# Rikorose/DeepFilterNet

Hardware: NVIDIA H100
Metric: 48kHz audio-sec/sec (batched enhance) (higher is better)
Workload: dtype f32 (bf16x3 tensor-core contractions, fp32 accumulate; DSP and gates IEEE fp32)

## Files before the change

### deepfilternet_b200/_lib.py

```python
from __future__ import annotations

import ctypes as C
import os
import subprocess

_HERE = os.path.dirname(os.path.abspath(__file__))
SO_PATH = os.path.join(_HERE, "libdfb200.so")

DFB_ERR_INVALID, DFB_ERR_CUDA, DFB_ERR_UNSUPPORTED, DFB_ERR_OOM = -1, -2, -3, -4


class DfbError(RuntimeError):
    def __init__(self, code: int, msg: str):
        super().__init__(msg)
        self.code = code


class ModelConfigC(C.Structure):
    _fields_ = [(n, C.c_int32) for n in (
        "model_kind", "nb_erb", "nb_df", "df_order", "df_lookahead", "conv_lookahead", "conv_ch",
        "conv_kt", "inp_kt", "emb_hidden", "df_hidden", "enc_gru_layers", "erb_gru_layers",
        "df_gru_layers", "df_pathway_kt", "enc_concat", "g_df_fc_emb", "g_enc_in", "g_enc_out",
        "g_erb_in", "g_erb_out", "g_df_in", "g_df_skip", "g_df_out")] + [
        ("lsnr_scale", C.c_float), ("lsnr_offset", C.c_float), ("norm_alpha", C.c_float)]


class TensorC(C.Structure):
    _fields_ = [("name", C.c_char_p), ("data", C.POINTER(C.c_float)), ("numel", C.c_int64)]


def build(force: bool = False) -> str:
    src_dir = os.path.join(_HERE, "csrc")
    if force and os.path.exists(SO_PATH):
        os.remove(SO_PATH)
    subprocess.check_call(["make", "-C", src_dir, "-j4"], stdout=subprocess.DEVNULL)
    return SO_PATH


_lib = None

_VP, _FP, _I64, _I, _F = C.c_void_p, C.POINTER(C.c_float), C.c_int64, C.c_int, C.c_float
_I64P = C.POINTER(C.c_int64)

SIGNATURES = {
    "dfb_last_error": (C.c_char_p, []),
    "dfb_version": (C.c_char_p, []),
    "dfb_kernel_launches": (_I64, []),
    "dfb_profile_enable": (_I, [_I, C.c_char_p]),
    "dfb_profile_report": (_I64, [C.c_char_p, _I64]),
    "dfb_state_create": (_I, [C.POINTER(_VP), _I, _I, _I, _I, _I, _I]),
    "dfb_state_free": (None, [_VP]),
    "dfb_state_erb_widths": (_I, [_VP, _I64P]),
    "dfb_state_fft_window": (_I, [_VP, _FP]),
    "dfb_state_params": (_I, [_VP, C.POINTER(_I), C.POINTER(_I), C.POINTER(_I), C.POINTER(_I)]),
    "dfb_erb_widths": (_I, [_I, _I, _I, _I, _I64P]),
    "dfb_analysis": (_I, [_VP, _VP, _I64, _I64, _VP, _VP]),
    "dfb_analysis_host": (_I, [_VP, _VP, _I64, _I64, _VP]),
    "dfb_analysis_host_ex": (_I, [_VP, _VP, _I64, _I64, _I, _VP]),
    "dfb_synthesis_host_ex": (_I, [_VP, _VP, _I64, _I64, _I, _VP]),
    "dfb_state_reset": (_I, [_VP]),
    "dfb_synthesis": (_I, [_VP, _VP, _I64, _I64, _VP, _VP]),
    "dfb_synthesis_host": (_I, [_VP, _VP, _I64, _I64, _VP]),
    "dfb_erb_host": (_I, [_I, _VP, _I64, _I64, _I64P, _I, _I, _VP]),
    "dfb_erb_inv_host": (_I, [_I, _VP, _I64, _I64P, _I, _VP]),
    "dfb_erb_norm_host": (_I, [_I, _VP, _I64, _I64, _I64, _F, _VP, _VP]),
    "dfb_unit_norm_host": (_I, [_I, _VP, _I64, _I64, _I64, _F, _VP, _VP]),
    "dfb_unit_norm_init": (_I, [_I64, _VP]),
    "dfb_features": (_I, [_VP, _VP, _I64, _I64, _I, _F, _VP, _VP, _VP, _VP]),
    "dfb_features_host": (_I, [_VP, _VP, _I64, _I64, _I, _F, _VP, _VP, _VP]),
    "dfb_resample_host": (_I, [_I, _VP, _I64, _I64, _VP, _I, _I, _I, _VP, _I64]),
    "dfb_model_create": (_I, [C.POINTER(_VP), _I, C.POINTER(ModelConfigC), C.POINTER(TensorC), _I, _I64P]),
    "dfb_model_free": (None, [_VP]),
    "dfb_model_forward": (_I, [_VP, _VP, _VP, _I64, _I64, _VP, _VP, _VP, _VP, _VP]),
    "dfb_apply": (_I, [_VP, _VP, _VP, _VP, _VP, _I64, _I64, _VP, _VP]),
    "dfb_model_forward_full": (_I, [_VP, _VP, _VP, _VP, _VP, _I64, _I64, _VP, _VP, _VP, _VP, _VP, _VP]),
    "dfb_enhance": (_I, [_VP, _VP, _VP, _I64, _I64, _I, _F, _VP, _VP]),
    "dfb_enhance_host": (_I, [_VP, _VP, _VP, _I64, _I64, _I, _F, _VP]),
    "dfb_enhance_out_len": (_I64, [_VP, _I64, _I]),
    "dfb_enhance_ragged": (_I, [_VP, _VP, _VP, _I64, _VP, _VP, _I64, _I, _F, _VP, _I64, _VP, _VP]),
    "dfb_enhance_ragged_host": (_I, [_VP, _VP, _VP, _I64, _VP, _VP, _I64, _I, _F, _VP, _I64, _VP]),
    "dfb_enhance_ragged_linked": (_I, [_VP, _VP, _VP, _I64, _VP, _VP, _I64, _I, _F, _VP, _I64, _VP, _VP, _I64, _I, _VP]),
    "dfb_enhance_ragged_linked_host": (_I, [_VP, _VP, _VP, _I64, _VP, _VP, _I64, _I, _F, _VP, _I64, _VP, _VP, _I64, _I]),
    "dfb_model_workspace_bytes": (_I64, [_VP]),
    "dfb_stream_create": (_I, [C.POINTER(_VP), _VP, _VP, _I64, _F]),
    "dfb_stream_free": (None, [_VP]),
    "dfb_stream_reset": (_I, [_VP]),
    "dfb_stream_frame_length": (_I64, [_VP]),
    "dfb_stream_latency_frames": (_I64, [_VP]),
    "dfb_stream_set_lsnr_thresholds": (_I, [_VP, _I, _F, _F, _F]),
    "dfb_stream_set_mask_reduce": (_I, [_VP, _I, _I]),
    "dfb_stream_process": (_I, [_VP, _VP, _I64, _VP, _VP]),
    "dfb_stream_flush": (_I, [_VP, _VP, _VP]),
    "dfb_stream_process_host": (_I, [_VP, _VP, _I64, _VP]),
    "dfb_stream_open_slots": (_I, [_VP, _I64P, _I64]),
    "dfb_stream_close_slots": (_I, [_VP, _I64P, _I64]),
    "dfb_stream_slot_states": (_I, [_VP, C.POINTER(C.c_int32)]),
    "dfb_stream_open_linked": (_I, [_VP, _I64P, _I64]),
    "dfb_stream_slot_groups": (_I, [_VP, _I64P]),
    "dfb_stream_set_atten_lim": (_I, [_VP, _I64P, _I64, _F]),
    "dfb_stream_set_post_filter_beta": (_I, [_VP, _I64P, _I64, _F]),
    "dfb_stream_process_lsnr": (_I, [_VP, _VP, _I64, _VP, _VP, _VP]),
    "dfb_stream_flush_lsnr": (_I, [_VP, _VP, _VP, _VP]),
    "dfb_stream_process_host_lsnr": (_I, [_VP, _VP, _I64, _VP, _VP]),
    "dfb_model_set_max_workspace": (_I, [_VP, _I64]),
    "dfb_model_set_options": (_I, [_VP, _I, _F, _I]),
    "dfb_model_set_chunking": (_I, [_VP, _I, _I, _I]),
    "dfb_debug_gru_timing": (_I, [_VP, _I, _VP]),
    "dfb_model_debug_fetch": (_I64, [_VP, C.c_char_p, _VP, _I64]),
}


def lib() -> C.CDLL:
    global _lib
    if _lib is None:
        if not os.path.exists(SO_PATH):
            raise ImportError(
                f"{SO_PATH} is missing: build it with `python -c 'import __graft_entry__ as g; g.build()'` "
                "(nvcc, sm_90a).  deepfilternet_b200 has no CPU fallback.")
        L = C.CDLL(SO_PATH)
        for name, (res, args) in SIGNATURES.items():
            fn = getattr(L, name)
            fn.restype = res
            fn.argtypes = args
        _lib = L
    return _lib


def check(rc: int) -> None:
    if rc != 0:
        msg = lib().dfb_last_error()
        raise DfbError(rc, (msg or b"unknown error").decode())
```

### deepfilternet_b200/csrc/dfb_gl.cu

```cuda
#include <cuda.h>
#include <cuda_bf16.h>

#include <map>
#include <mutex>
#include <tuple>

#include "dfb_common.cuh"
#include "dfb_dwpw.cuh"
#include "dfb_ptx.cuh"

namespace dfb {

constexpr int kGxThreads = 288, kGxMaxStages = 6, kGxBoxBytes = 128 * 128 ;
constexpr int kGxMaxChunks = 16;

struct GlBxParams {
    const unsigned short *w_img;
    const float *res; int64_t ldr;
    float *y; int64_t ldy;
    unsigned short *y_hi, *y_lo; int64_t ldp;
    int M, G, Ig, Hg, Hgp, gpc, act, stages;
    float oscale, ooffset;
};

__device__ __forceinline__ float gx_act(float x, int act) {
    if (act == 1) return fmaxf(x, 0.f);
    if (act == 2) return gt_tanh(x);
    return x;
}

__device__ __noinline__ void gl_store_chunk(const GlBxParams &p, int c, int g0, int cpg, int64_t mrow, int lane, float a00, float a01,
                                            float a02, float a03, float a10, float a11, float a12, float a13) {
    const float a[2][4] = {{a00, a01, a02, a03}, {a10, a11, a12, a13}};
    const int gl = c / cpg;
#pragma unroll
    for (int j = 0; j < 2; j++) {
        const int n = (c - gl * cpg) * 16 + j * 8 + 2 * (lane & 3);
        if (n >= p.Hg) continue;
        const int64_t col = (int64_t)(g0 + gl) * p.Hg + n;
        float2 rv[2];
#pragma unroll
        for (int h = 0; h < 2; h++) {
            const int64_t m = mrow + 8 * h;
            rv[h] = (p.res && m < p.M) ? *reinterpret_cast<const float2 *>(p.res + m * p.ldr + col) : make_float2(0.f, 0.f);
        }
#pragma unroll
        for (int h = 0; h < 2; h++) {
            const int64_t m = mrow + 8 * h;
            if (m >= p.M) continue;
            float2 x;
            x.x = gx_act(a[j][2 * h], p.act) * p.oscale + p.ooffset + rv[h].x;
            x.y = gx_act(a[j][2 * h + 1], p.act) * p.oscale + p.ooffset + rv[h].y;
            if (p.y) *reinterpret_cast<float2 *>(p.y + m * p.ldy + col) = x;
            if (p.y_hi) {
                uint32_t hv, lv;
                bf16x2_split(x.x, x.y, hv, lv);
                *reinterpret_cast<uint32_t *>(p.y_hi + m * p.ldp + col) = hv;
                *reinterpret_cast<uint32_t *>(p.y_lo + m * p.ldp + col) = lv;
            }
        }
    }
}

__global__ void __launch_bounds__(kGxThreads, 1)
k_gl_bx(const __grid_constant__ CUtensorMap tmXhi, const __grid_constant__ CUtensorMap tmXlo, const __grid_constant__ GlBxParams p) {
    extern __shared__ __align__(1024) unsigned char gx_smem_raw[];
    const uint32_t sb = (smem_u32(gx_smem_raw) + 1023u) & ~1023u;
    const int warp = threadIdx.x >> 5, lane = threadIdx.x & 31;
    const int slice = blockIdx.x, g0 = slice * p.gpc;
    const int nch = p.gpc * p.Hgp / 16;
    const int cpg = p.Hgp / 16;
    const int nboxes = p.gpc * p.Ig / 64;
    const int ntiles = (p.M + 127) / 128;
    const uint32_t gbytes = (uint32_t)p.Ig * p.Hgp * 2;
    const uint32_t wplane = gbytes * p.gpc;
    const uint32_t lbo = (uint32_t)(p.Hgp / 8) * 128u;
    const uint32_t s_x = sb;
    const uint32_t s_w = s_x + (uint32_t)p.stages * 2 * kGxBoxBytes;
    const uint32_t s_bar = (s_w + 2 * wplane + 127u) & ~127u;
    const uint32_t b_full = s_bar, b_empty = s_bar + 8 * kGxMaxStages, b_w = b_empty + 8 * kGxMaxStages;
    if (threadIdx.x == 0) {
        for (int s = 0; s < p.stages; s++) { mbar_init_a(b_full + 8 * s, 1); mbar_init_a(b_empty + 8 * s, 8); }
        mbar_init_a(b_w, 1);
        fence_barrier_init();
        mbar_expect_tx_a(b_w, 2 * wplane);
        const unsigned char *src = reinterpret_cast<const unsigned char *>(p.w_img);
        bulk_load(s_w, src + (size_t)g0 * gbytes, wplane, b_w);
        bulk_load(s_w + wplane, src + (size_t)p.G * gbytes + (size_t)g0 * gbytes, wplane, b_w);
    }
    __syncthreads();
    if (warp == 8) {
        if (lane == 0) {
            tma_prefetch_desc(&tmXhi); tma_prefetch_desc(&tmXlo);
            const int col0 = g0 * p.Ig;
            int it = 0;
            for (int tile = blockIdx.y; tile < ntiles; tile += gridDim.y)
                for (int b = 0; b < nboxes; b++, it++) {
                    const int s = it % p.stages, n = it / p.stages;
                    if (n > 0) mbar_wait_a(b_empty + 8 * s, (uint32_t)((n - 1) & 1));
                    mbar_expect_tx_a(b_full + 8 * s, 2 * kGxBoxBytes);
                    const uint32_t dst = s_x + (uint32_t)s * 2 * kGxBoxBytes;
                    asm volatile(
                        "cp.async.bulk.tensor.2d.shared::cluster.global.mbarrier::complete_tx::bytes [%0], [%1, {%2, %3}], [%4];"
                        ::"r"(dst), "l"((uint64_t)&tmXhi), "r"(col0 + b * 64), "r"(tile * 128), "r"(b_full + 8 * s) : "memory");
                    asm volatile(
                        "cp.async.bulk.tensor.2d.shared::cluster.global.mbarrier::complete_tx::bytes [%0], [%1, {%2, %3}], [%4];"
                        ::"r"(dst + kGxBoxBytes), "l"((uint64_t)&tmXlo), "r"(col0 + b * 64), "r"(tile * 128), "r"(b_full + 8 * s) : "memory");
                }
        }
        return;
    }
    const int mat = lane >> 3, rr = lane & 7;
    mbar_wait_a(b_w, 0);
    int it = 0;
    for (int tile = blockIdx.y; tile < ntiles; tile += gridDim.y) {
        float acc[kGxMaxChunks][2][4];
#pragma unroll
        for (int c = 0; c < kGxMaxChunks; c++)
#pragma unroll
            for (int e = 0; e < 8; e++) acc[c][e >> 2][e & 3] = 0.f;
        for (int b = 0; b < nboxes; b++, it++) {
            const int s = it % p.stages, n = it / p.stages;
            mbar_wait_a(b_full + 8 * s, (uint32_t)(n & 1));
            const uint32_t xs = s_x + (uint32_t)s * 2 * kGxBoxBytes;
#pragma unroll 1
            for (int k = 0; k < 4; k++) {
                const int col = b * 64 + k * 16;
                const int gl = col / p.Ig, kk = (col - gl * p.Ig) >> 4;
                uint32_t ah[4], al[4];
                const int r = warp * 16 + rr + ((mat & 1) << 3);
                ldsm_x4(xs + sw128_off(r, 2 * k + (mat >> 1)), ah);
                ldsm_x4(xs + kGxBoxBytes + sw128_off(r, 2 * k + (mat >> 1)), al);
                const uint32_t wa = s_w + (uint32_t)gl * gbytes + (uint32_t)(2 * kk + (mat & 1)) * lbo + (uint32_t)rr * 16u;
#pragma unroll
                for (int c = 0; c < kGxMaxChunks; c++) {
                    const int cg = c - gl * cpg;
                    if (c >= nch || cg < 0 || cg >= cpg) continue;
                    const uint32_t o = wa + (uint32_t)(2 * cg + (mat >> 1)) * 128u;
                    uint32_t bh[4], bl[4];
                    ldsm_x4(o, bh);
                    ldsm_x4(o + wplane, bl);
                    mma_bf16x3(acc[c][0], ah, al, bh[0], bh[1], bl[0], bl[1]);
                    mma_bf16x3(acc[c][1], ah, al, bh[2], bh[3], bl[2], bl[3]);
                }
            }
            __syncwarp();
            if (lane == 0) mbar_arrive_a(b_empty + 8 * s);
        }
        const int64_t mrow = (int64_t)tile * 128 + warp * 16 + (lane >> 2);
#pragma unroll
        for (int c = 0; c < kGxMaxChunks; c++)
            if (c < nch)
                gl_store_chunk(p, c, g0, cpg, mrow, lane, acc[c][0][0], acc[c][0][1], acc[c][0][2], acc[c][0][3], acc[c][1][0],
                               acc[c][1][1], acc[c][1][2], acc[c][1][3]);
    }
}

constexpr int kDeThreads = 288, kDeMaxStages = 6, kDeMaxChunks = 4;
constexpr uint32_t kDeBin = 32768;

struct DfEmbParams {
    const float *dw;
    const float *bias;
    const float *pw_sw;
    const unsigned short *w_img;
    const float *res; int64_t ldr;
    unsigned short *y_hi, *y_lo; int64_t ldp;
    int M, T, G, Ig, Hg, Hgp, S, stages;
    float oscale, ooffset;
    const int64_t *first;
    int64_t w0;
};

template <int KT>
__global__ void __launch_bounds__(kDeThreads, 1)
k_dwpw_gl(const __grid_constant__ CUtensorMap tmC0, const __grid_constant__ DfEmbParams p) {
    extern __shared__ __align__(1024) unsigned char de_smem_raw[];
    const uint32_t sb = (smem_u32(de_smem_raw) + 1023u) & ~1023u;
    const int warp = threadIdx.x >> 5, lane = threadIdx.x & 31;
    constexpr int RT = 128 - (KT - 1);
    const int ntiles = (p.M + RT - 1) / RT;
    const int j0 = blockIdx.x * p.S;
    const int f_lo = j0 > 0 ? 2 * j0 - 1 : 0, f_hi = 2 * (j0 + p.S);
    const int gps = p.S * kCh / p.Ig, cpg = p.Hgp / 16, nch = gps * cpg;
    const int g0 = j0 * kCh / p.Ig;
    const uint32_t gbytes = (uint32_t)p.Ig * p.Hgp * 2;
    const uint32_t wplane = gbytes * gps;
    const uint32_t lbo = (uint32_t)(p.Hgp / 8) * 128u;
    const uint32_t s_c0 = sb;
    const uint32_t s_pw = s_c0 + (uint32_t)p.stages * kDeBin;
    const uint32_t s_w = s_pw + 2u * kCh * 128u;
    const uint32_t s_bias = s_w + 2 * wplane;
    const uint32_t s_dw = s_bias + 256u;
    const uint32_t s_bar = (s_dw + KT * 3 * kCh * 4u + 127u) & ~127u;
    const uint32_t b_full = s_bar, b_empty = s_bar + 8 * kDeMaxStages, b_w = b_empty + 8 * kDeMaxStages;
    if (threadIdx.x == 0) {
        for (int s = 0; s < p.stages; s++) { mbar_init_a(b_full + 8 * s, 1); mbar_init_a(b_empty + 8 * s, 8); }
        mbar_init_a(b_w, 1);
        fence_barrier_init();
        mbar_expect_tx_a(b_w, 2u * kCh * 128u + 2 * wplane);
        bulk_load(s_pw, p.pw_sw, 2u * kCh * 128u, b_w);
        const unsigned char *src = reinterpret_cast<const unsigned char *>(p.w_img);
        bulk_load(s_w, src + (size_t)g0 * gbytes, wplane, b_w);
        bulk_load(s_w + wplane, src + (size_t)p.G * gbytes + (size_t)g0 * gbytes, wplane, b_w);
    }
    if (threadIdx.x < kCh / 4) sts128(s_bias + threadIdx.x * 16, __ldg(reinterpret_cast<const float4 *>(p.bias) + threadIdx.x));
    for (int i = threadIdx.x; i < KT * 3 * kCh / 4; i += kDeThreads) sts128(s_dw + i * 16, __ldg(reinterpret_cast<const float4 *>(p.dw) + i));
    __syncthreads();
    if (warp == 8) {
        if (lane == 0) {
            tma_prefetch_desc(&tmC0);
            int it = 0;
            for (int tile = blockIdx.y; tile < ntiles; tile += gridDim.y) {
                const int row0 = tile * RT - (KT - 1);
                for (int f = f_lo; f < f_hi; f++, it++) {
                    const int s = it % p.stages, n = it / p.stages;
                    if (n > 0) mbar_wait_a(b_empty + 8 * s, (uint32_t)((n - 1) & 1));
                    mbar_expect_tx_a(b_full + 8 * s, kDeBin);
                    const uint32_t dst = s_c0 + (uint32_t)s * kDeBin;
                    asm volatile(
                        "cp.async.bulk.tensor.2d.shared::cluster.global.mbarrier::complete_tx::bytes [%0], [%1, {%2, %3}], [%4];"
                        ::"r"(dst), "l"((uint64_t)&tmC0), "r"(f * kCh), "r"(row0), "r"(b_full + 8 * s) : "memory");
                    asm volatile(
                        "cp.async.bulk.tensor.2d.shared::cluster.global.mbarrier::complete_tx::bytes [%0], [%1, {%2, %3}], [%4];"
                        ::"r"(dst + kDeBin / 2), "l"((uint64_t)&tmC0), "r"(f * kCh + 32), "r"(row0), "r"(b_full + 8 * s) : "memory");
                }
            }
        }
        return;
    }
    const int g = lane >> 2, q = lane & 3, mat = lane >> 3, rr = lane & 7;
    mbar_wait_a(b_w, 0);
    int it = 0;
    for (int tile = blockIdx.y; tile < ntiles; tile += gridDim.y, it += f_hi - f_lo) {
        const int row0 = tile * RT - (KT - 1);
        bool tap_ok[2][KT];
#pragma unroll
        for (int rs = 0; rs < 2; rs++) {
            const int r = warp * 16 + g + 8 * rs, m = row0 + r;
#pragma unroll
            for (int dt = 0; dt < KT; dt++) tap_ok[rs][dt] = true;
            if (KT > 1) {
                const int b = m >= 0 && m < p.M ? m / p.T : 0, t = m - b * p.T;
                const int t_first = stream_first(p.first, b, p.w0);
#pragma unroll
                for (int dt = 0; dt < KT; dt++) tap_ok[rs][dt] = r - (KT - 1) + dt >= 0 && t - (KT - 1 - dt) >= t_first;
            }
        }
        float gacc[kDeMaxChunks][2][4];
#pragma unroll
        for (int c = 0; c < kDeMaxChunks; c++)
#pragma unroll
            for (int e = 0; e < 8; e++) gacc[c][e >> 2][e & 3] = 0.f;
        for (int jj = 0; jj < p.S; jj++) {
            const int j = j0 + jj;
            uint32_t slot[3];
#pragma unroll
            for (int df = 0; df < 3; df++) {
                const int f = 2 * j - 1 + df;
                const int i = it + (f < f_lo ? 0 : f - f_lo);
                slot[df] = s_c0 + (uint32_t)(i % p.stages) * kDeBin;
                if (f >= f_lo) mbar_wait_a(b_full + 8 * (i % p.stages), (uint32_t)((i / p.stages) & 1));
            }
            uint32_t ah[4][4], al[4][4];
#pragma unroll
            for (int ks = 0; ks < 4; ks++)
#pragma unroll
                for (int h = 0; h < 2; h++) {
                    const int ch = 16 * ks + 8 * h + 2 * q;
                    const uint32_t cbase = (uint32_t)(ch >> 5) * (kDeBin / 2) + (uint32_t)(ch & 3) * 4u;
                    const int chunk = (ch & 31) >> 2;
#pragma unroll
                    for (int rs = 0; rs < 2; rs++) {
                        const int r = warp * 16 + g + 8 * rs;
                        float2 acc = make_float2(0.f, 0.f);
#pragma unroll
                        for (int dt = 0; dt < KT; dt++) {
                            if (!tap_ok[rs][dt]) continue;
                            const int rb = r - (KT - 1) + dt;
                            const uint32_t o = cbase + (uint32_t)rb * 128u + (uint32_t)((chunk ^ (rb & 7)) << 4);
#pragma unroll
                            for (int df = 0; df < 3; df++) {
                                if (df == 0 && j == 0) continue;
                                float2 x;
                                asm volatile("ld.shared.v2.f32 {%0, %1}, [%2];" : "=f"(x.x), "=f"(x.y) : "r"(slot[df] + o));
                                float2 w;
                                asm volatile("ld.shared.v2.f32 {%0, %1}, [%2];" : "=f"(w.x), "=f"(w.y) : "r"(s_dw + 4u * ((dt * 3 + df) * kCh + ch)));
                                acc.x = fmaf(x.x, w.x, acc.x);
                                acc.y = fmaf(x.y, w.y, acc.y);
                            }
                        }
                        bf16x2_split(acc.x, acc.y, ah[ks][rs + 2 * h], al[ks][rs + 2 * h]);
                    }
                }
            __syncwarp();
            if (lane == 0) {
                for (int f = 2 * j - 1; f <= 2 * j + (jj + 1 == p.S ? 1 : 0); f++)
                    if (f >= f_lo) mbar_arrive_a(b_empty + 8 * ((it + f - f_lo) % p.stages));
            }
            float acc[8][4];
#pragma unroll
            for (int nt = 0; nt < 8; nt++)
#pragma unroll
                for (int e = 0; e < 4; e++) acc[nt][e] = 0.f;
#pragma unroll
            for (int ks = 0; ks < 4; ks++)
#pragma unroll
                for (int np = 0; np < 4; np++) {
                    const int n = 16 * np + rr + ((mat >> 1) << 3);
                    const uint32_t o = sw128_off(n, 2 * ks + (mat & 1));
                    uint32_t bh[4], bl[4];
                    ldsm_x4(s_pw + o, bh);
                    ldsm_x4(s_pw + 8192 + o, bl);
                    mma_bf16x3(acc[2 * np], ah[ks], al[ks], bh[0], bh[1], bl[0], bl[1]);
                    mma_bf16x3(acc[2 * np + 1], ah[ks], al[ks], bh[2], bh[3], bl[2], bl[3]);
                }
            uint32_t ch_[4][4], cl_[4][4];
#pragma unroll
            for (int nt = 0; nt < 8; nt++) {
                const int c = 8 * nt + 2 * q;
                float b0, b1;
                asm volatile("ld.shared.v2.f32 {%0, %1}, [%2];" : "=f"(b0), "=f"(b1) : "r"(s_bias + 4 * c));
#pragma unroll
                for (int rs = 0; rs < 2; rs++)
                    bf16x2_split(fmaxf(acc[nt][2 * rs] + b0, 0.f), fmaxf(acc[nt][2 * rs + 1] + b1, 0.f), ch_[nt >> 1][rs + 2 * (nt & 1)],
                                 cl_[nt >> 1][rs + 2 * (nt & 1)]);
            }
#pragma unroll
            for (int kk = 0; kk < 4; kk++) {
                const int col = jj * kCh + kk * 16;
                const int gl = col / p.Ig, kq = (col - gl * p.Ig) >> 4;
                const uint32_t wa = s_w + (uint32_t)gl * gbytes + (uint32_t)(2 * kq + (mat & 1)) * lbo + (uint32_t)rr * 16u;
#pragma unroll
                for (int c = 0; c < kDeMaxChunks; c++) {
                    const int cg = c - gl * cpg;
                    if (c >= nch || cg < 0 || cg >= cpg) continue;
                    const uint32_t o = wa + (uint32_t)(2 * cg + (mat >> 1)) * 128u;
                    uint32_t bh[4], bl[4];
                    ldsm_x4(o, bh);
                    ldsm_x4(o + wplane, bl);
                    mma_bf16x3(gacc[c][0], ch_[kk], cl_[kk], bh[0], bh[1], bl[0], bl[1]);
                    mma_bf16x3(gacc[c][1], ch_[kk], cl_[kk], bh[2], bh[3], bl[2], bl[3]);
                }
            }
        }
        const int64_t mrow = (int64_t)row0 + warp * 16 + g;
        const int64_t mmin = (int64_t)tile * RT;
#pragma unroll
        for (int c = 0; c < kDeMaxChunks; c++) {
            if (c >= nch) continue;
            const int gl = c / cpg;
#pragma unroll
            for (int jh = 0; jh < 2; jh++) {
                const int n = (c - gl * cpg) * 16 + jh * 8 + 2 * q;
                if (n >= p.Hg) continue;
                const int64_t col = (int64_t)(g0 + gl) * p.Hg + n;
                float2 rv[2];
#pragma unroll
                for (int rs = 0; rs < 2; rs++) {
                    const int64_t m = mrow + 8 * rs;
                    rv[rs] = (p.res && m >= mmin && m < p.M) ? *reinterpret_cast<const float2 *>(p.res + m * p.ldr + col) : make_float2(0.f, 0.f);
                }
#pragma unroll
                for (int rs = 0; rs < 2; rs++) {
                    const int64_t m = mrow + 8 * rs;
                    if (m < mmin || m >= p.M) continue;
                    float2 x;
                    x.x = gx_act(gacc[c][jh][2 * rs], 1) * p.oscale + p.ooffset + rv[rs].x;
                    x.y = gx_act(gacc[c][jh][2 * rs + 1], 1) * p.oscale + p.ooffset + rv[rs].y;
                    uint32_t hv, lv;
                    bf16x2_split(x.x, x.y, hv, lv);
                    *reinterpret_cast<uint32_t *>(p.y_hi + m * p.ldp + col) = hv;
                    *reinterpret_cast<uint32_t *>(p.y_lo + m * p.ldp + col) = lv;
                }
            }
        }
    }
}

__global__ void __launch_bounds__(256) k_to_planes(const float *__restrict__ x, int64_t ldx, int64_t M, int K,
                                                   unsigned short *__restrict__ hi, unsigned short *__restrict__ lo) {
    const int64_t n4 = M * (K / 4);
    for (int64_t i = (int64_t)blockIdx.x * blockDim.x + threadIdx.x; i < n4; i += (int64_t)gridDim.x * blockDim.x) {
        const int64_t m = i / (K / 4);
        const int k = (int)(i - m * (K / 4)) * 4;
        const float4 v = *reinterpret_cast<const float4 *>(x + m * ldx + k);
        uint32_t h0, l0, h1, l1;
        bf16x2_split(v.x, v.y, h0, l0);
        bf16x2_split(v.z, v.w, h1, l1);
        *reinterpret_cast<uint2 *>(hi + m * K + k) = make_uint2(h0, h1);
        *reinterpret_cast<uint2 *>(lo + m * K + k) = make_uint2(l0, l1);
    }
}

typedef CUresult (*PFN_encodeTiled_gl)(CUtensorMap *, CUtensorMapDataType, cuuint32_t, void *, const cuuint64_t *,
                                       const cuuint64_t *, const cuuint32_t *, const cuuint32_t *, CUtensorMapInterleave,
                                       CUtensorMapSwizzle, CUtensorMapL2promotion, CUtensorMapFloatOOBfill);

int cached_map_bf16(CUtensorMap *out, const void *base, int64_t rows, int64_t cols, int64_t ld, int box_rows) {
    static std::mutex mu;
    static std::map<std::tuple<int, const void *, int64_t, int64_t, int64_t, int>, CUtensorMap> cache;
    static PFN_encodeTiled_gl enc = nullptr;
    int dev = 0;
    cudaGetDevice(&dev);
    std::lock_guard<std::mutex> g(mu);
    auto key = std::make_tuple(dev, base, rows, cols, ld, box_rows);
    auto it = cache.find(key);
    if (it != cache.end()) { *out = it->second; return DFB_OK; }
    if (!enc) {
        void *fp = nullptr;
        cudaDriverEntryPointQueryResult q;
        if (cudaGetDriverEntryPoint("cuTensorMapEncodeTiled", &fp, cudaEnableDefault, &q) != cudaSuccess || q != cudaDriverEntryPointSuccess)
            return fail(DFB_ERR_CUDA, "cuTensorMapEncodeTiled entry point not available");
        enc = (PFN_encodeTiled_gl)fp;
    }
    cuuint64_t dims[2] = {(cuuint64_t)cols, (cuuint64_t)rows};
    cuuint64_t strides[1] = {(cuuint64_t)ld * 2};
    cuuint32_t box[2] = {64u, (cuuint32_t)box_rows};
    cuuint32_t estr[2] = {1, 1};
    CUtensorMap m;
    CUresult r = enc(&m, CU_TENSOR_MAP_DATA_TYPE_BFLOAT16, 2, (void *)base, dims, strides, box, estr, CU_TENSOR_MAP_INTERLEAVE_NONE,
                     CU_TENSOR_MAP_SWIZZLE_128B, CU_TENSOR_MAP_L2_PROMOTION_L2_128B, CU_TENSOR_MAP_FLOAT_OOB_FILL_NONE);
    if (r != CUDA_SUCCESS) return fail(DFB_ERR_CUDA, "cuTensorMapEncodeTiled (bf16) failed (%d)", (int)r);
    if (cache.size() > 4096) cache.clear();
    cache[key] = m;
    *out = m;
    return DFB_OK;
}

int cached_map_f32_sw128(CUtensorMap *out, const void *base, int64_t rows, int64_t cols, int64_t ld, int box_rows) {
    static std::mutex mu;
    static std::map<std::tuple<int, const void *, int64_t, int64_t, int64_t, int>, CUtensorMap> cache;
    static PFN_encodeTiled_gl enc = nullptr;
    int dev = 0;
    cudaGetDevice(&dev);
    std::lock_guard<std::mutex> g(mu);
    auto key = std::make_tuple(dev, base, rows, cols, ld, box_rows);
    auto it = cache.find(key);
    if (it != cache.end()) { *out = it->second; return DFB_OK; }
    if (!enc) {
        void *fp = nullptr;
        cudaDriverEntryPointQueryResult q;
        if (cudaGetDriverEntryPoint("cuTensorMapEncodeTiled", &fp, cudaEnableDefault, &q) != cudaSuccess || q != cudaDriverEntryPointSuccess)
            return fail(DFB_ERR_CUDA, "cuTensorMapEncodeTiled entry point not available");
        enc = (PFN_encodeTiled_gl)fp;
    }
    cuuint64_t dims[2] = {(cuuint64_t)cols, (cuuint64_t)rows};
    cuuint64_t strides[1] = {(cuuint64_t)ld * 4};
    cuuint32_t box[2] = {32u, (cuuint32_t)box_rows};
    cuuint32_t estr[2] = {1, 1};
    CUtensorMap m;
    CUresult r = enc(&m, CU_TENSOR_MAP_DATA_TYPE_FLOAT32, 2, (void *)base, dims, strides, box, estr, CU_TENSOR_MAP_INTERLEAVE_NONE,
                     CU_TENSOR_MAP_SWIZZLE_128B, CU_TENSOR_MAP_L2_PROMOTION_L2_128B, CU_TENSOR_MAP_FLOAT_OOB_FILL_NONE);
    if (r != CUDA_SUCCESS) return fail(DFB_ERR_CUDA, "cuTensorMapEncodeTiled (fp32) failed (%d)", (int)r);
    if (cache.size() > 4096) cache.clear();
    cache[key] = m;
    *out = m;
    return DFB_OK;
}

int launch_to_planes(cudaStream_t s, const float *x, int64_t ldx, int64_t M, int K, unsigned short *hi, unsigned short *lo) {
    if (K % 4 || ldx % 4) return fail(DFB_ERR_UNSUPPORTED, "to_planes: K = %d", K);
    int dev = 0, sms = 0;
    DFB_CUDA(cudaGetDevice(&dev));
    DFB_CUDA(cudaDeviceGetAttribute(&sms, cudaDevAttrMultiProcessorCount, dev));
    DFB_PROF("k_to_planes", s);
    k_to_planes<<<sms * 8, 256, 0, s>>>(x, ldx, M, K, hi, lo);
    DFB_LAUNCH_CHECK();
    return DFB_OK;
}

bool gl_bx_geometry(int G, int Ig, int Hg, int *gpc_out, int *hgp_out, int *stages_out) {
    if (Ig % 16 || Hg % 4 || G < 1) return false;
    const int Hgp = (Hg + 15) / 16 * 16;
    if (Hgp > 256) return false;
    int best = 0;
    for (int gpc = 1; gpc <= G; gpc++) {
        if (G % gpc) continue;
        if (gpc * Hgp > 256 || (gpc * Hgp) % 32) continue;
        if ((gpc * Ig) % 64) continue;
        if ((size_t)gpc * Ig * Hgp * 4 > 100 * 1024) continue;
        best = gpc;
    }
    if (!best) return false;
    const int w = best * Ig * Hgp * 4;
    int stages = (227 * 1024 - 2048 - w - 256) / (2 * kGxBoxBytes);
    if (stages > kGxMaxStages) stages = kGxMaxStages;
    if (stages < 2) return false;
    *gpc_out = best; *hgp_out = Hgp; *stages_out = stages;
    return true;
}

int launch_gl_bx(cudaStream_t s, const unsigned short *x_hi, const unsigned short *x_lo, int64_t ldx, const float *w_img,
                 const float *res, int64_t ldr, float *y, int64_t ldy, unsigned short *y_hi, unsigned short *y_lo, int64_t ldp,
                 int64_t M, int G, int Ig, int Hg, int act, float oscale, float ooffset) {
    int gpc = 0, Hgp = 0, stages = 0;
    if (!gl_bx_geometry(G, Ig, Hg, &gpc, &Hgp, &stages) || M <= 0 || M > 0x7fffffff || (ldx % 8) || ((uintptr_t)x_hi & 15) ||
        ((uintptr_t)x_lo & 15) || (y && ((ldy % 4) || ((uintptr_t)y & 15))) || (res && ((ldr % 4) || ((uintptr_t)res & 15))) ||
        (y_hi && ((ldp % 4) || ((uintptr_t)y_hi & 7) || ((uintptr_t)y_lo & 7))))
        return DFB_ERR_UNSUPPORTED;
    CUtensorMap mh, ml;
    int rc;
    if ((rc = cached_map_bf16(&mh, x_hi, M, (int64_t)G * Ig, ldx, 128)) || (rc = cached_map_bf16(&ml, x_lo, M, (int64_t)G * Ig, ldx, 128)))
        return rc;
    GlBxParams p{reinterpret_cast<const unsigned short *>(w_img), res, ldr, y, ldy, y_hi, y_lo, ldp,
                 (int)M, G, Ig, Hg, Hgp, gpc, act, stages, oscale, ooffset};
    const int smem = 1024 + stages * 2 * kGxBoxBytes + gpc * Ig * Hgp * 4 + 128 + 256;
    static PerDeviceOnce attr_once;
    if (auto once_guard = attr_once.first())
        DFB_CUDA(cudaFuncSetAttribute(k_gl_bx, cudaFuncAttributeMaxDynamicSharedMemorySize, 227 * 1024));
    int dev = 0, sms = 0;
    DFB_CUDA(cudaGetDevice(&dev));
    DFB_CUDA(cudaDeviceGetAttribute(&sms, cudaDevAttrMultiProcessorCount, dev));
    const int slices = G / gpc, ntiles = (int)((M + 127) / 128);
    int groups = sms / slices;
    if (groups < 1) groups = 1;
    if (groups > ntiles) groups = ntiles;
    DFB_PROF("k_gl_bx", s);
    k_gl_bx<<<dim3((unsigned)slices, (unsigned)groups), kGxThreads, smem, s>>>(mh, ml, p);
    DFB_LAUNCH_CHECK();
    return DFB_OK;
}

bool df_emb_geometry(int Fd, int G, int Ig, int Hg, int kt, int *s_out, int *stages_out) {
    if ((kt != 1 && kt != 2) || Fd % 2 || Ig % 16 || Hg % 4 || G < 1 || G * Ig != Fd / 2 * kCh) return false;
    int S = 1;
    while ((S * kCh) % Ig) S++;
    const int Hgp = (Hg + 15) / 16 * 16;
    if ((Fd / 2) % S || (S * kCh / Ig) * (Hgp / 16) > kDeMaxChunks) return false;
    const int fixed = 1024 + 2 * kCh * 128 + S * kCh * Hgp * 4 + 256 + kt * 3 * kCh * 4 + 128 + 2 * 8 * kDeMaxStages + 8;
    int stages = (227 * 1024 - fixed) / (int)kDeBin;
    if (stages > kDeMaxStages) stages = kDeMaxStages;
    if (stages < 3) return false;
    *s_out = S; *stages_out = stages;
    return true;
}

int launch_df_emb(cudaStream_t s, const float *c0, int64_t M, int T, int Fd, int kt, const float *dw, const float *bias,
                  const float *pw_sw, const float *w_img, int G, int Ig, int Hg, const float *res, int64_t ldr,
                  unsigned short *y_hi, unsigned short *y_lo, int64_t ldp, const int64_t *first, int64_t w0) {
    int S = 0, stages = 0;
    if (!df_emb_geometry(Fd, G, Ig, Hg, kt, &S, &stages) || M <= 0 || M > 0x7fffffff - 256 || T <= 0 || M % T ||
        (res && ((ldr % 2) || ((uintptr_t)res & 7))) || (ldp % 2) || ((uintptr_t)y_hi & 3) || ((uintptr_t)y_lo & 3) ||
        ((uintptr_t)c0 & 15) || ((uintptr_t)w_img & 15) || ((uintptr_t)pw_sw & 15))
        return fail(DFB_ERR_UNSUPPORTED, "df_conv1 + df_fc_emb kernel: shape G %d Ig %d Hg %d kt %d", G, Ig, Hg, kt);
    CUtensorMap mc;
    int rc;
    if ((rc = cached_map_f32_sw128(&mc, c0, M, (int64_t)Fd * kCh, (int64_t)Fd * kCh, 128))) return rc;
    const int Hgp = (Hg + 15) / 16 * 16;
    DfEmbParams p{dw, bias, pw_sw, reinterpret_cast<const unsigned short *>(w_img), res, ldr, y_hi, y_lo, ldp,
                  (int)M, T, G, Ig, Hg, Hgp, S, stages, 1.f, 0.f, first, w0};
    const int smem = 1024 + stages * (int)kDeBin + 2 * kCh * 128 + S * kCh * Hgp * 4 + 256 + kt * 3 * kCh * 4 + 128 + 2 * 8 * kDeMaxStages + 8;
    static PerDeviceOnce attr_once;
    if (auto once_guard = attr_once.first()) {
        DFB_CUDA(cudaFuncSetAttribute(k_dwpw_gl<1>, cudaFuncAttributeMaxDynamicSharedMemorySize, 227 * 1024));
        DFB_CUDA(cudaFuncSetAttribute(k_dwpw_gl<2>, cudaFuncAttributeMaxDynamicSharedMemorySize, 227 * 1024));
    }
    int dev = 0, sms = 0;
    DFB_CUDA(cudaGetDevice(&dev));
    DFB_CUDA(cudaDeviceGetAttribute(&sms, cudaDevAttrMultiProcessorCount, dev));
    const int slices = Fd / 2 / S, rt = 128 - (kt - 1);
    const int ntiles = (int)((M + rt - 1) / rt);
    int groups = sms / slices;
    if (groups < 1) groups = 1;
    if (groups > ntiles) groups = ntiles;
    DFB_PROF("k_dwpw_gl", s);
    if (kt == 1) k_dwpw_gl<1><<<dim3((unsigned)slices, (unsigned)groups), kDeThreads, smem, s>>>(mc, p);
    else k_dwpw_gl<2><<<dim3((unsigned)slices, (unsigned)groups), kDeThreads, smem, s>>>(mc, p);
    DFB_LAUNCH_CHECK();
    return DFB_OK;
}

}
```

### include/dfb200.h

```cpp
#ifndef DFB200_H
#define DFB200_H

#include <stdint.h>

#ifdef __cplusplus
extern "C" {
#endif

typedef enum {
    DFB_OK = 0,
    DFB_ERR_INVALID = -1,
    DFB_ERR_CUDA = -2,
    DFB_ERR_UNSUPPORTED = -3,
    DFB_ERR_OOM = -4
} dfb_status;

const char *dfb_last_error(void);
const char *dfb_version(void);
int64_t dfb_kernel_launches(void);

int dfb_profile_enable(int on, const char *only_kernel);
int64_t dfb_profile_report(char *buf, int64_t buflen);

typedef struct dfb_state dfb_state;

int dfb_state_create(dfb_state **out, int device, int sr, int fft_size, int hop_size, int nb_erb,
                     int min_nb_erb_freqs);
void dfb_state_free(dfb_state *st);
int dfb_state_erb_widths(const dfb_state *st, int64_t *widths );
int dfb_state_fft_window(const dfb_state *st, float *window );
int dfb_state_params(const dfb_state *st, int *sr, int *fft_size, int *hop_size, int *nb_erb);
int dfb_erb_widths(int sr, int fft_size, int nb_erb, int min_nb_freqs, int64_t *widths);

int dfb_analysis(dfb_state *st, const float *d_audio, int64_t C, int64_t T, float *d_spec, void *stream);
int dfb_analysis_host(dfb_state *st, const float *h_audio, int64_t C, int64_t T, float *h_spec);
int dfb_analysis_host_ex(dfb_state *st, const float *h_audio, int64_t C, int64_t T, int reset, float *h_spec);
int dfb_state_reset(dfb_state *st);

int dfb_synthesis(dfb_state *st, const float *d_spec, int64_t C, int64_t Tf, float *d_audio, void *stream);
int dfb_synthesis_host(dfb_state *st, const float *h_spec, int64_t C, int64_t Tf, float *h_audio);
int dfb_synthesis_host_ex(dfb_state *st, const float *h_spec, int64_t C, int64_t Tf, int reset, float *h_audio);

int dfb_erb_host(int device, const float *h_spec, int64_t n_frames, int64_t F, const int64_t *widths, int E,
                 int db, float *h_out);
int dfb_erb_inv_host(int device, const float *h_gains, int64_t n_frames, const int64_t *widths, int E,
                     float *h_out );
int dfb_erb_norm_host(int device, const float *h_erb, int64_t C, int64_t T, int64_t E, float alpha,
                      const float *h_state, float *h_out);
int dfb_unit_norm_host(int device, const float *h_spec, int64_t C, int64_t T, int64_t F, float alpha,
                       const float *h_state, float *h_out);
int dfb_unit_norm_init(int64_t n, float *h_out);

int dfb_features(dfb_state *st, const float *d_audio, int64_t C, int64_t T, int nb_df, float alpha,
                 float *d_spec, float *d_feat_erb, float *d_feat_spec, void *stream);
int dfb_features_host(dfb_state *st, const float *h_audio, int64_t C, int64_t T, int nb_df, float alpha,
                      float *h_spec, float *h_feat_erb, float *h_feat_spec);

int dfb_resample_host(int device, const float *h_audio, int64_t C, int64_t T, const float *h_kernel, int orig, int new_rate,
                      int width, float *h_out, int64_t T_out);

typedef struct dfb_model dfb_model;

typedef struct {
    int32_t model_kind;
    int32_t nb_erb, nb_df, df_order, df_lookahead, conv_lookahead;
    int32_t conv_ch;
    int32_t conv_kt;
    int32_t inp_kt;
    int32_t emb_hidden, df_hidden;
    int32_t enc_gru_layers, erb_gru_layers, df_gru_layers;
    int32_t df_pathway_kt;
    int32_t enc_concat;
    int32_t g_df_fc_emb, g_enc_in, g_enc_out, g_erb_in, g_erb_out, g_df_in, g_df_skip, g_df_out;
    float lsnr_scale, lsnr_offset;
    float norm_alpha;
} dfb_model_config;

typedef struct {
    const char *name;
    const float *data;
    int64_t numel;
} dfb_tensor;

int dfb_model_create(dfb_model **out, int device, const dfb_model_config *cfg, const dfb_tensor *tensors,
                     int n_tensors, const int64_t *erb_widths);
void dfb_model_free(dfb_model *m);

int dfb_model_forward(dfb_model *m, const float *d_feat_erb, const float *d_feat_spec, int64_t B, int64_t T,
                      float *d_m, float *d_coefs, float *d_lsnr, float *d_alpha, void *stream);

int dfb_apply(dfb_model *m, dfb_state *st, const float *d_spec, const float *d_m, const float *d_coefs,
              int64_t B, int64_t T, float *d_spec_e, void *stream);

int dfb_model_forward_full(dfb_model *m, dfb_state *st, const float *d_spec, const float *d_feat_erb,
                           const float *d_feat_spec, int64_t B, int64_t T, float *d_spec_e, float *d_m,
                           float *d_lsnr, float *d_coefs, float *d_alpha, void *stream);

int dfb_enhance(dfb_model *m, dfb_state *st, const float *d_audio, int64_t B, int64_t T, int pad,
                float atten_lim_db, float *d_out, void *stream);
int dfb_enhance_host(dfb_model *m, dfb_state *st, const float *h_audio, int64_t B, int64_t T, int pad,
                     float atten_lim_db, float *h_out);
int64_t dfb_enhance_out_len(const dfb_state *st, int64_t T, int pad);
int dfb_enhance_ragged(dfb_model *m, dfb_state *st, const float *d_audio, int64_t in_numel, const int64_t *in_offsets,
                       const int64_t *lengths, int64_t B, int pad, float atten_lim_db, float *d_out, int64_t out_numel,
                       const int64_t *out_offsets, void *stream);
int dfb_enhance_ragged_host(dfb_model *m, dfb_state *st, const float *h_audio, int64_t in_numel, const int64_t *in_offsets,
                            const int64_t *lengths, int64_t B, int pad, float atten_lim_db, float *h_out, int64_t out_numel,
                            const int64_t *out_offsets);
typedef enum { DFB_REDUCE_NONE = 0, DFB_REDUCE_MAX = 1, DFB_REDUCE_MEAN = 2 } dfb_reduce_mask;
int dfb_enhance_ragged_linked(dfb_model *m, dfb_state *st, const float *d_audio, int64_t in_numel, const int64_t *in_offsets,
                              const int64_t *lengths, int64_t B, int pad, float atten_lim_db, float *d_out, int64_t out_numel,
                              const int64_t *out_offsets, const int64_t *group_sizes, int64_t n_groups, int reduce_mask,
                              void *stream);
int dfb_enhance_ragged_linked_host(dfb_model *m, dfb_state *st, const float *h_audio, int64_t in_numel,
                                   const int64_t *in_offsets, const int64_t *lengths, int64_t B, int pad, float atten_lim_db,
                                   float *h_out, int64_t out_numel, const int64_t *out_offsets, const int64_t *group_sizes,
                                   int64_t n_groups, int reduce_mask);
typedef struct dfb_stream dfb_stream;
int dfb_stream_create(dfb_stream **out, dfb_model *m, dfb_state *st, int64_t B, float atten_lim_db);
void dfb_stream_free(dfb_stream *s);
int dfb_stream_reset(dfb_stream *s);
int64_t dfb_stream_frame_length(const dfb_stream *s);
int64_t dfb_stream_latency_frames(const dfb_stream *s);
int dfb_stream_set_lsnr_thresholds(dfb_stream *s, int enable, float min_db_thresh, float max_db_erb_thresh,
                                   float max_db_df_thresh);
int dfb_stream_set_mask_reduce(dfb_stream *s, int channels, int reduce_mask);
int dfb_stream_process(dfb_stream *s, const float *d_in, int64_t n_frames, float *d_out, void *stream);
int dfb_stream_flush(dfb_stream *s, float *d_out, void *stream);
int dfb_stream_process_host(dfb_stream *s, const float *h_in, int64_t n_frames, float *h_out);

int dfb_stream_open_slots(dfb_stream *s, const int64_t *slots, int64_t n);
int dfb_stream_close_slots(dfb_stream *s, const int64_t *slots, int64_t n);
int dfb_stream_slot_states(const dfb_stream *s, int32_t *h_states);
int dfb_stream_open_linked(dfb_stream *s, const int64_t *slots, int64_t n);
int dfb_stream_slot_groups(const dfb_stream *s, int64_t *h_first);

int dfb_stream_set_atten_lim(dfb_stream *s, const int64_t *slots, int64_t n, float atten_lim_db);
int dfb_stream_set_post_filter_beta(dfb_stream *s, const int64_t *slots, int64_t n, float beta);

int dfb_stream_process_lsnr(dfb_stream *s, const float *d_in, int64_t n_frames, float *d_out, float *d_lsnr, void *stream);
int dfb_stream_flush_lsnr(dfb_stream *s, float *d_out, float *d_lsnr, void *stream);
int dfb_stream_process_host_lsnr(dfb_stream *s, const float *h_in, int64_t n_frames, float *h_out, float *h_lsnr);

int dfb_model_set_chunking(dfb_model *m, int device_chunks, int host_chunks, int lanes);
int dfb_model_set_options(dfb_model *m, int post_filter, float pf_beta, int mask_only);
int dfb_model_set_max_workspace(dfb_model *m, int64_t bytes);
int dfb_debug_gru_timing(dfb_model *m, int steps, long long *h_out);
int64_t dfb_model_debug_fetch(dfb_model *m, const char *name, float *h_out, int64_t max_numel);
int64_t dfb_model_workspace_bytes(const dfb_model *m);

#ifdef __cplusplus
}
#endif
#endif
```

Before: 64590.

## Stage grouped-linear output and residual through shared memory with TMA stores

```diff
diff --git a/deepfilternet_b200/_lib.py b/deepfilternet_b200/_lib.py
--- a/deepfilternet_b200/_lib.py
+++ b/deepfilternet_b200/_lib.py
@@ -106,6 +106,7 @@
     "dfb_model_set_options": (_I, [_VP, _I, _F, _I]),
     "dfb_model_set_chunking": (_I, [_VP, _I, _I, _I]),
     "dfb_debug_gru_timing": (_I, [_VP, _I, _VP]),
+    "dfb_debug_gl_bx": (_I, [_VP, _VP, _I64, _VP, _VP, _I64, _VP, _I64, _VP, _VP, _I64, _I64, _I, _I, _I, _I, _F, _F, _VP]),
     "dfb_model_debug_fetch": (_I64, [_VP, C.c_char_p, _VP, _I64]),
 }
 
diff --git a/deepfilternet_b200/csrc/dfb_gl.cu b/deepfilternet_b200/csrc/dfb_gl.cu
--- a/deepfilternet_b200/csrc/dfb_gl.cu
+++ b/deepfilternet_b200/csrc/dfb_gl.cu
@@ -21,6 +21,7 @@
     unsigned short *y_hi, *y_lo; int64_t ldp;
     int M, G, Ig, Hg, Hgp, gpc, act, stages;
     float oscale, ooffset;
+    int stage_y;
 };
 
 __device__ __forceinline__ float gx_act(float x, int act) {
@@ -29,10 +30,38 @@
     return x;
 }
 
-__device__ __noinline__ void gl_store_chunk(const GlBxParams &p, int c, int g0, int cpg, int64_t mrow, int lane, float a00, float a01,
-                                            float a02, float a03, float a10, float a11, float a12, float a13) {
+__device__ __noinline__ void gl_store_chunk(const GlBxParams &p, int c, int g0, int cpg, int64_t mrow, int lane, uint32_t st,
+                                            float a00, float a01, float a02, float a03, float a10, float a11, float a12, float a13) {
     const float a[2][4] = {{a00, a01, a02, a03}, {a10, a11, a12, a13}};
     const int gl = c / cpg;
+    if (st) {
+        const uint32_t pitch = (uint32_t)(p.gpc * p.Hg) * 4u;
+#pragma unroll
+        for (int j = 0; j < 2; j++) {
+            const int n = (c - gl * cpg) * 16 + j * 8 + 2 * (lane & 3);
+            if (n >= p.Hg) continue;
+            const int lcol = gl * p.Hg + n;
+            const int64_t col = (int64_t)g0 * p.Hg + lcol;
+#pragma unroll
+            for (int h = 0; h < 2; h++) {
+                const uint32_t sa = st + (uint32_t)((lane >> 2) + 8 * h) * pitch + (uint32_t)lcol * 4u;
+                float2 rv = make_float2(0.f, 0.f);
+                if (p.res) asm volatile("ld.shared.v2.f32 {%0, %1}, [%2];" : "=f"(rv.x), "=f"(rv.y) : "r"(sa));
+                float2 x;
+                x.x = gx_act(a[j][2 * h], p.act) * p.oscale + p.ooffset + rv.x;
+                x.y = gx_act(a[j][2 * h + 1], p.act) * p.oscale + p.ooffset + rv.y;
+                sts64(sa, __float_as_uint(x.x), __float_as_uint(x.y));
+                const int64_t m = mrow + 8 * h;
+                if (p.y_hi && m < p.M) {
+                    uint32_t hv, lv;
+                    bf16x2_split(x.x, x.y, hv, lv);
+                    *reinterpret_cast<uint32_t *>(p.y_hi + m * p.ldp + col) = hv;
+                    *reinterpret_cast<uint32_t *>(p.y_lo + m * p.ldp + col) = lv;
+                }
+            }
+        }
+        return;
+    }
 #pragma unroll
     for (int j = 0; j < 2; j++) {
         const int n = (c - gl * cpg) * 16 + j * 8 + 2 * (lane & 3);
@@ -63,7 +92,8 @@
 }
 
 __global__ void __launch_bounds__(kGxThreads, 1)
-k_gl_bx(const __grid_constant__ CUtensorMap tmXhi, const __grid_constant__ CUtensorMap tmXlo, const __grid_constant__ GlBxParams p) {
+k_gl_bx(const __grid_constant__ CUtensorMap tmXhi, const __grid_constant__ CUtensorMap tmXlo, const __grid_constant__ CUtensorMap tmY,
+        const __grid_constant__ CUtensorMap tmR, const __grid_constant__ GlBxParams p) {
     extern __shared__ __align__(1024) unsigned char gx_smem_raw[];
     const uint32_t sb = (smem_u32(gx_smem_raw) + 1023u) & ~1023u;
     const int warp = threadIdx.x >> 5, lane = threadIdx.x & 31;
@@ -77,11 +107,16 @@
     const uint32_t lbo = (uint32_t)(p.Hgp / 8) * 128u;
     const uint32_t s_x = sb;
     const uint32_t s_w = s_x + (uint32_t)p.stages * 2 * kGxBoxBytes;
-    const uint32_t s_bar = (s_w + 2 * wplane + 127u) & ~127u;
+    const uint32_t ybox = 16u * (uint32_t)(p.gpc * p.Hg) * 4u;
+    const uint32_t s_y = s_w + 2 * wplane;
+    const uint32_t s_bar = (s_y + (p.stage_y ? 8 * ybox : 0u) + 127u) & ~127u;
     const uint32_t b_full = s_bar, b_empty = s_bar + 8 * kGxMaxStages, b_w = b_empty + 8 * kGxMaxStages;
+    const uint32_t b_rfull = b_w + 8, b_rempty = b_rfull + 8 * 8;
+    const bool res_tma = p.stage_y && p.res;
     if (threadIdx.x == 0) {
         for (int s = 0; s < p.stages; s++) { mbar_init_a(b_full + 8 * s, 1); mbar_init_a(b_empty + 8 * s, 8); }
         mbar_init_a(b_w, 1);
+        for (int w = 0; w < 8; w++) { mbar_init_a(b_rfull + 8 * w, 1); mbar_init_a(b_rempty + 8 * w, 1); }
         fence_barrier_init();
         mbar_expect_tx_a(b_w, 2 * wplane);
         const unsigned char *src = reinterpret_cast<const unsigned char *>(p.w_img);
@@ -92,9 +127,10 @@
     if (warp == 8) {
         if (lane == 0) {
             tma_prefetch_desc(&tmXhi); tma_prefetch_desc(&tmXlo);
+            if (res_tma) tma_prefetch_desc(&tmR);
             const int col0 = g0 * p.Ig;
-            int it = 0;
-            for (int tile = blockIdx.y; tile < ntiles; tile += gridDim.y)
+            int it = 0, ti = 0;
+            for (int tile = blockIdx.y; tile < ntiles; tile += gridDim.y, ti++) {
                 for (int b = 0; b < nboxes; b++, it++) {
                     const int s = it % p.stages, n = it / p.stages;
                     if (n > 0) mbar_wait_a(b_empty + 8 * s, (uint32_t)((n - 1) & 1));
@@ -107,13 +143,23 @@
                         "cp.async.bulk.tensor.2d.shared::cluster.global.mbarrier::complete_tx::bytes [%0], [%1, {%2, %3}], [%4];"
                         ::"r"(dst + kGxBoxBytes), "l"((uint64_t)&tmXlo), "r"(col0 + b * 64), "r"(tile * 128), "r"(b_full + 8 * s) : "memory");
                 }
+                for (int w = 0; res_tma && w < 8; w++) {
+                    if (ti > 0) mbar_wait_a(b_rempty + 8 * w, (uint32_t)((ti - 1) & 1));
+                    mbar_expect_tx_a(b_rfull + 8 * w, ybox);
+                    asm volatile(
+                        "cp.async.bulk.tensor.2d.shared::cluster.global.mbarrier::complete_tx::bytes [%0], [%1, {%2, %3}], [%4];"
+                        ::"r"(s_y + (uint32_t)w * ybox), "l"((uint64_t)&tmR), "r"(g0 * p.Hg), "r"(tile * 128 + 16 * w), "r"(b_rfull + 8 * w)
+                        : "memory");
+                }
+            }
         }
         return;
     }
     const int mat = lane >> 3, rr = lane & 7;
     mbar_wait_a(b_w, 0);
-    int it = 0;
-    for (int tile = blockIdx.y; tile < ntiles; tile += gridDim.y) {
+    const uint32_t st = p.stage_y ? s_y + (uint32_t)warp * ybox : 0u;
+    int it = 0, ti = 0;
+    for (int tile = blockIdx.y; tile < ntiles; tile += gridDim.y, ti++) {
         float acc[kGxMaxChunks][2][4];
 #pragma unroll
         for (int c = 0; c < kGxMaxChunks; c++)
@@ -148,11 +194,24 @@
             if (lane == 0) mbar_arrive_a(b_empty + 8 * s);
         }
         const int64_t mrow = (int64_t)tile * 128 + warp * 16 + (lane >> 2);
+        if (res_tma) mbar_wait_a(b_rfull + 8 * warp, (uint32_t)(ti & 1));
 #pragma unroll
         for (int c = 0; c < kGxMaxChunks; c++)
             if (c < nch)
-                gl_store_chunk(p, c, g0, cpg, mrow, lane, acc[c][0][0], acc[c][0][1], acc[c][0][2], acc[c][0][3], acc[c][1][0],
+                gl_store_chunk(p, c, g0, cpg, mrow, lane, st, acc[c][0][0], acc[c][0][1], acc[c][0][2], acc[c][0][3], acc[c][1][0],
                                acc[c][1][1], acc[c][1][2], acc[c][1][3]);
+        if (st) {
+            fence_proxy_async();
+            __syncwarp();
+            if (lane == 0) {
+                asm volatile("cp.async.bulk.tensor.2d.global.shared::cta.bulk_group [%0, {%1, %2}], [%3];"
+                             ::"l"((uint64_t)&tmY), "r"(g0 * p.Hg), "r"(tile * 128 + warp * 16), "r"(st) : "memory");
+                asm volatile("cp.async.bulk.commit_group;" ::: "memory");
+                asm volatile("cp.async.bulk.wait_group.read 0;" ::: "memory");
+                if (res_tma) mbar_arrive_a(b_rempty + 8 * warp);
+            }
+            __syncwarp();
+        }
     }
 }
 
@@ -459,6 +518,37 @@
     return DFB_OK;
 }
 
+static int cached_map_f32_rows(CUtensorMap *out, const void *base, int64_t rows, int64_t cols, int64_t ld, int box_cols, int box_rows) {
+    static std::mutex mu;
+    static std::map<std::tuple<int, const void *, int64_t, int64_t, int64_t, int, int>, CUtensorMap> cache;
+    static PFN_encodeTiled_gl enc = nullptr;
+    int dev = 0;
+    cudaGetDevice(&dev);
+    std::lock_guard<std::mutex> g(mu);
+    auto key = std::make_tuple(dev, base, rows, cols, ld, box_cols, box_rows);
+    auto it = cache.find(key);
+    if (it != cache.end()) { *out = it->second; return DFB_OK; }
+    if (!enc) {
+        void *fp = nullptr;
+        cudaDriverEntryPointQueryResult q;
+        if (cudaGetDriverEntryPoint("cuTensorMapEncodeTiled", &fp, cudaEnableDefault, &q) != cudaSuccess || q != cudaDriverEntryPointSuccess)
+            return fail(DFB_ERR_CUDA, "cuTensorMapEncodeTiled entry point not available");
+        enc = (PFN_encodeTiled_gl)fp;
+    }
+    cuuint64_t dims[2] = {(cuuint64_t)cols, (cuuint64_t)rows};
+    cuuint64_t strides[1] = {(cuuint64_t)ld * 4};
+    cuuint32_t box[2] = {(cuuint32_t)box_cols, (cuuint32_t)box_rows};
+    cuuint32_t estr[2] = {1, 1};
+    CUtensorMap m;
+    CUresult r = enc(&m, CU_TENSOR_MAP_DATA_TYPE_FLOAT32, 2, (void *)base, dims, strides, box, estr, CU_TENSOR_MAP_INTERLEAVE_NONE,
+                     CU_TENSOR_MAP_SWIZZLE_NONE, CU_TENSOR_MAP_L2_PROMOTION_L2_128B, CU_TENSOR_MAP_FLOAT_OOB_FILL_NONE);
+    if (r != CUDA_SUCCESS) return fail(DFB_ERR_CUDA, "cuTensorMapEncodeTiled (fp32 rows) failed (%d)", (int)r);
+    if (cache.size() > 4096) cache.clear();
+    cache[key] = m;
+    *out = m;
+    return DFB_OK;
+}
+
 int launch_to_planes(cudaStream_t s, const float *x, int64_t ldx, int64_t M, int K, unsigned short *hi, unsigned short *lo) {
     if (K % 4 || ldx % 4) return fail(DFB_ERR_UNSUPPORTED, "to_planes: K = %d", K);
     int dev = 0, sms = 0;
@@ -503,9 +593,19 @@
     int rc;
     if ((rc = cached_map_bf16(&mh, x_hi, M, (int64_t)G * Ig, ldx, 128)) || (rc = cached_map_bf16(&ml, x_lo, M, (int64_t)G * Ig, ldx, 128)))
         return rc;
+    const int wbytes = gpc * Ig * Hgp * 4, ybytes = 128 * gpc * Hg * 4;
+    int stages_y = (227 * 1024 - 2048 - wbytes - ybytes - 256) / (2 * kGxBoxBytes);
+    if (stages_y > kGxMaxStages) stages_y = kGxMaxStages;
+    const bool stage_y = y && stages_y >= 2;
+    CUtensorMap my = mh, mr = mh;
+    if (stage_y) {
+        stages = stages_y;
+        if ((rc = cached_map_f32_rows(&my, y, M, (int64_t)G * Hg, ldy, gpc * Hg, 16))) return rc;
+        if (res && (rc = cached_map_f32_rows(&mr, res, M, (int64_t)G * Hg, ldr, gpc * Hg, 16))) return rc;
+    }
     GlBxParams p{reinterpret_cast<const unsigned short *>(w_img), res, ldr, y, ldy, y_hi, y_lo, ldp,
-                 (int)M, G, Ig, Hg, Hgp, gpc, act, stages, oscale, ooffset};
-    const int smem = 1024 + stages * 2 * kGxBoxBytes + gpc * Ig * Hgp * 4 + 128 + 256;
+                 (int)M, G, Ig, Hg, Hgp, gpc, act, stages, oscale, ooffset, stage_y ? 1 : 0};
+    const int smem = 1024 + stages * 2 * kGxBoxBytes + wbytes + (stage_y ? ybytes : 0) + 128 + 256;
     static PerDeviceOnce attr_once;
     if (auto once_guard = attr_once.first())
         DFB_CUDA(cudaFuncSetAttribute(k_gl_bx, cudaFuncAttributeMaxDynamicSharedMemorySize, 227 * 1024));
@@ -517,10 +617,24 @@
     if (groups < 1) groups = 1;
     if (groups > ntiles) groups = ntiles;
     DFB_PROF("k_gl_bx", s);
-    k_gl_bx<<<dim3((unsigned)slices, (unsigned)groups), kGxThreads, smem, s>>>(mh, ml, p);
+    k_gl_bx<<<dim3((unsigned)slices, (unsigned)groups), kGxThreads, smem, s>>>(mh, ml, my, mr, p);
     DFB_LAUNCH_CHECK();
     return DFB_OK;
 }
+
+}
+
+extern "C" int dfb_debug_gl_bx(const void *x_hi, const void *x_lo, int64_t ldx, const float *w_img, const float *res, int64_t ldr,
+                               float *y, int64_t ldy, void *y_hi, void *y_lo, int64_t ldp, int64_t M, int G, int Ig, int Hg,
+                               int act, float oscale, float ooffset, void *stream) {
+    if (!x_hi || !x_lo || !w_img || (!y && !y_hi) || (!y_hi != !y_lo)) return dfb::fail(DFB_ERR_INVALID, "gl_bx: null argument");
+    const int r = dfb::launch_gl_bx((cudaStream_t)stream, (const unsigned short *)x_hi, (const unsigned short *)x_lo, ldx, w_img, res,
+                                    ldr, y, ldy, (unsigned short *)y_hi, (unsigned short *)y_lo, ldp, M, G, Ig, Hg, act, oscale, ooffset);
+    if (r == DFB_ERR_UNSUPPORTED) return dfb::fail(r, "gl_bx: shape G %d Ig %d Hg %d or pointer alignment not built", G, Ig, Hg);
+    return r;
+}
+
+namespace dfb {
 
 bool df_emb_geometry(int Fd, int G, int Ig, int Hg, int kt, int *s_out, int *stages_out) {
     if ((kt != 1 && kt != 2) || Fd % 2 || Ig % 16 || Hg % 4 || G < 1 || G * Ig != Fd / 2 * kCh) return false;
diff --git a/include/dfb200.h b/include/dfb200.h
--- a/include/dfb200.h
+++ b/include/dfb200.h
@@ -146,6 +146,9 @@
 int dfb_model_set_options(dfb_model *m, int post_filter, float pf_beta, int mask_only);
 int dfb_model_set_max_workspace(dfb_model *m, int64_t bytes);
 int dfb_debug_gru_timing(dfb_model *m, int steps, long long *h_out);
+int dfb_debug_gl_bx(const void *x_hi, const void *x_lo, int64_t ldx, const float *w_img, const float *res, int64_t ldr,
+                    float *y, int64_t ldy, void *y_hi, void *y_lo, int64_t ldp, int64_t M, int G, int Ig, int Hg, int act,
+                    float oscale, float ooffset, void *stream);
 int64_t dfb_model_debug_fetch(dfb_model *m, const char *name, float *h_out, int64_t max_numel);
 int64_t dfb_model_workspace_bytes(const dfb_model *m);
 
```

After: 69030, median of 6. 1.07x the previous value.
